# SimLeek/pySILEnT

Measured on AMD Instinct MI355X. Metric: Mpx/s full pyramid line-end pass @1080p, 1/2/4/8 GPU; % HBM roofline, higher is better.
Workload: dtype f32

## Files before the change

pysilent_amd/csrc/silent_common.h:

```cpp
#pragma once

#include <hip/hip_runtime.h>
#include <stdint.h>

#include <type_traits>

#include "../../include/silent_hip.h"

namespace silent {

constexpr int kMaxLevels = SILENT_MAX_LEVELS;
constexpr int kWave = 64;

struct LevelTab {
    int n_levels;
    int tiles_per_frame;
    long long frame_px;
    int h[kMaxLevels];
    int w[kMaxLevels];
    int tiles_x[kMaxLevels];
    int tile_start[kMaxLevels + 1];
    long long px_off[kMaxLevels];
};

constexpr int kChunk = 1024;

struct TileCoord {
    int frame, level, ty, tx;
};

__device__ __forceinline__ unsigned xcd_swizzle(unsigned bid, unsigned n) {
    constexpr unsigned kXcd = 8;
    const unsigned per = n / kXcd, rem = n % kXcd;
    const unsigned x = bid % kXcd, k = bid / kXcd;
    return x * per + (x < rem ? x : rem) + k;
}

__device__ __forceinline__ TileCoord locate_tile(const LevelTab& tab, unsigned bid) {
    TileCoord t;
    t.frame = (int)(bid / (unsigned)tab.tiles_per_frame);
    int rem = (int)(bid - (unsigned)t.frame * (unsigned)tab.tiles_per_frame);
    int l = 0;
#pragma unroll
    for (int i = 1; i < kMaxLevels; ++i)
        if (i < tab.n_levels && rem >= tab.tile_start[i]) l = i;
    t.level = l;
    rem -= tab.tile_start[l];
    t.ty = rem / tab.tiles_x[l];
    t.tx = rem - t.ty * tab.tiles_x[l];
    return t;
}

__device__ __forceinline__ float from_lane_below(float v) {
    return __int_as_float(__builtin_amdgcn_update_dpp(0, __float_as_int(v), 0x138 , 0xf, 0xf, true));
}
__device__ __forceinline__ float from_lane_above(float v) {
    return __int_as_float(__builtin_amdgcn_update_dpp(0, __float_as_int(v), 0x130 , 0xf, 0xf, true));
}

template <bool F64>
using acc_t = typename std::conditional<F64, double, float>::type;
__device__ __forceinline__ double bpermute_f64(int addr, double v) {
    return __hiloint2double(__builtin_amdgcn_ds_bpermute(addr, __double2hiint(v)), __builtin_amdgcn_ds_bpermute(addr, __double2loint(v)));
}

constexpr int kMirrorNearMin = 5;
__device__ __forceinline__ int mirror_near(int i, int n) {
    i = i < 0 ? -i : i;
    i = i >= n ? 2 * (n - 1) - i : i;
    return min(max(i, 0), n - 1);
}

template <bool EDGE = true>
__device__ __forceinline__ float unit_taps6(float c0, float edge, const float (&w)[6]) {
    const float l1 = from_lane_below(c0), l2 = from_lane_below(l1);
    float r1;
    if constexpr (EDGE)
        r1 = __int_as_float(__builtin_amdgcn_update_dpp(__float_as_int(edge), __float_as_int(c0), 0x130 , 0xf, 0xf, false));
    else
        r1 = from_lane_above(c0);
    const float r2 = from_lane_above(r1), r3 = from_lane_above(r2);
    float h = w[0] * l2;
    h = __builtin_fmaf(w[1], l1, h);
    h = __builtin_fmaf(w[2], c0, h);
    h = __builtin_fmaf(w[3], r1, h);
    h = __builtin_fmaf(w[4], r2, h);
    return __builtin_fmaf(w[5], r3, h);
}
template <bool EDGE = true>
__device__ __forceinline__ double unit_taps6(float c0, float edge, const double (&w)[6]) {
// ... 139 lines not shown
```

pysilent_amd/csrc/silent_gray.h:

```cpp
#pragma once

#include "silent_common.h"

namespace silent {

struct GrayW {
    float cs[9];
    float end[9 * 8];
};

constexpr int kGrayCols = 60;
constexpr int kGrayTW = 4 * kGrayCols;
constexpr int kGrayTH = 16;

template <bool NT = false>
__device__ __forceinline__ void store_row_k8(float* __restrict__ row_base ,
                                             const float (&acc)[8], float* s_slab ,
                                             int lane, int first, int count) {
    typedef float nf4 __attribute__((ext_vector_type(4)));
    nf4* slab4 = reinterpret_cast<nf4*>(s_slab);
    slab4[lane * 2 + 0] = nf4{acc[0], acc[1], acc[2], acc[3]};
    slab4[lane * 2 + 1] = nf4{acc[4], acc[5], acc[6], acc[7]};
    __builtin_amdgcn_wave_barrier();
    const nf4 a = slab4[lane], b = slab4[64 + lane];
// ... 42 lines not shown
#define SILENT_F16_CS_PAIRED 1
#endif
template <bool NT>
__device__ __forceinline__ void store_cs_row(gray_half* __restrict__ row0, float v, int lane, int first, int count) {
    const gray_half h = (gray_half)v;
    const unsigned mine = (unsigned)__builtin_bit_cast(unsigned short, h);
    const bool own = lane >= first && lane < first + count;
#if SILENT_F16_CS_PAIRED
    const unsigned up = (unsigned)__builtin_amdgcn_update_dpp(0, (int)mine, 0x130 , 0xf, 0xf, true);
    const int odd0 = (int)((reinterpret_cast<unsigned long long>(row0) >> 1) & 1ull);
    const bool lead = ((lane + odd0) & 1) == 0;
    const bool pair = own && lead && lane + 1 < first + count;
    const bool single = own && (lead ? lane + 1 >= first + count : lane == first);
    if (pair) {
        unsigned* p = reinterpret_cast<unsigned*>(row0 + lane);
        if constexpr (NT) __builtin_nontemporal_store(mine | (up << 16), p);
        else *p = mine | (up << 16);
    }
    if (single) {
        unsigned short* p = reinterpret_cast<unsigned short*>(row0 + lane);
        if constexpr (NT) __builtin_nontemporal_store((unsigned short)mine, p);
        else *p = (unsigned short)mine;
    }
#else
    if (own) {
        unsigned short* p = reinterpret_cast<unsigned short*>(row0 + lane);
        if constexpr (NT) __builtin_nontemporal_store((unsigned short)mine, p);
        else *p = (unsigned short)mine;
    }
#endif
}
template <typename ST>
constexpr bool kStoreHalf = std::is_same<ST, gray_half>::value;

struct GrayKp {
    unsigned* mm;
    float* sum;
    int* nan_flags;
    float* value_out;
    long long sum_frame;
    long long sum_off[kMaxLevels];
    int n_levels, pad, gpt;
    int level[kMaxLevels];
};

struct GrayKpAcc {
    float mx = kPoolLowest, nmn = kPoolLowest, grp = kPoolLowest;
    bool nan = false;
};

template <int K>
__device__ __forceinline__ void gray_kp_pixel(const GrayKp& kp, const float (&acc)[K], int y, int x, int H, int W, bool valid,
                                              float* __restrict__ value_px, GrayKpAcc& a) {
    const float m = (y >= kp.pad && y < H - kp.pad && x >= kp.pad && x < W - kp.pad) ? 1.0f : 0.0f;
    float s = __fmul_rn(m, acc[0]);
#pragma unroll
    for (int k = 1; k < K; ++k) s = __fadd_rn(s, __fmul_rn(m, acc[k]));
    const float v = __fmul_rn(s, 1.0f / (float)K);
    if (valid) {
        a.mx = pool_max(a.mx, v);
        a.nmn = pool_max(a.nmn, -v);
        a.grp = pool_max(a.grp, v);
        a.nan = a.nan || v != v;
        if (kp.value_out) *value_px = v;
    }
}
// ... 446 lines not shown
    if constexpr (F64) return stream_col64(st, g, wx_tile, lane);
    else return stream_col(st, g, wx_tile, lane);
}
template <int L, int G, int GR, int PR>
__device__ __forceinline__ void stream_level_f64(int g, const int (&cur)[PR], float c0, double (&vacc)[kStreamSlots],
                                                 const StreamCol64 (&col)[GR > 0 ? GR : 1], const StreamTab& st, int wx_tile, int lane,
                                                 float* __restrict__ pyr, long long frame_px0, int C, int ch) {
    const int meta = cur[g];
#pragma unroll
    for (int k = 0; k < stream_slots(L, g); ++k) {
        const int e = stream_w_off(L, G, g, true) + 2 * k;
        const double w = __hiloint2double(cur[e + 1], cur[e]);
        const double prev = (meta >> k) & 1 ? 0.0 : vacc[k];
        vacc[k] = __builtin_fma(w, (double)c0, prev);
    }
    const int done = (meta >> stream_done_shift(L)) & 7;
    if (done != 7) {
        const int oy = meta >> stream_row_shift(L);
        double v = vacc[0];
#pragma unroll
        for (int k = 1; k < stream_slots(L, g); ++k) v = done == k ? vacc[k] : v;
        const StreamCol64 cr = g < GR ? col[g < GR ? g : 0] : stream_col64(st, g, wx_tile, lane);
        double acc = cr.w[0] * bpermute_f64(cr.lane4, v);
#pragma unroll
        for (int t = 1; t < 6; ++t) acc = __builtin_fma(cr.w[t], bpermute_f64(cr.lane4 + 4 * t, v), acc);
        if (lane < cr.n) pyr[(frame_px0 + st.px_off[g] + (long long)oy * st.out_w[g] + cr.x0 + lane) * C + ch] = (float)acc;
    }
}
#ifndef SILENT_STREAM_REG_LEVELS
#define SILENT_STREAM_REG_LEVELS 3
#endif
constexpr int kStreamRegLevels = SILENT_STREAM_REG_LEVELS;

template <int K, int G, int L = 0, bool KP = false, bool F64 = false, typename ST = float, typename FT = float>
__global__ __launch_bounds__(64 * kFusedWaves) void gray_stream_kernel(frame_param<FT> frames, float* __restrict__ pyr,
                                                          ST* __restrict__ cs_out, ST* __restrict__ end_out,
                                                          const FusedTabT<F64> tab, const StreamTab st, const GrayW wts,
                                                          float clip_hi, unsigned opts, const GrayKp kp = GrayKp{}) {
    constexpr int R = kFusedTH, NR = kStreamRows;
    static_assert(!kStoreHalf<ST> || (!KP && !F64), "float16 storage: no keypoint epilogue, no float64 accumulation");
    static_assert(kFrameType<FT> && (!kFrameNarrow<FT> || !F64), "uint8 / uint16 frames: float32 accumulation only");
    __shared__ __attribute__((aligned(16))) float s_slab[K == 8 && !kStoreHalf<ST> ? kFusedWaves * 512 : 4];
    __shared__ __attribute__((aligned(16))) float s_rows[kFusedWaves][NR][64];
    const unsigned bid = (opts & 1u) ? xcd_swizzle(blockIdx.x, gridDim.x) : blockIdx.x;
    const int frame = (int)(bid / (unsigned)tab.tiles_per_frame);
    const int rem = (int)(bid - (unsigned)frame * (unsigned)tab.tiles_per_frame);
    const FusedLevel& lv = tab.lv[0];
    const int ty = rem / lv.tiles_x, tx = rem - ty * lv.tiles_x;

    const int lane = threadIdx.x & 63;
    const int wave = __builtin_amdgcn_readfirstlane(threadIdx.x >> 6);
    const int xw0 = tx * kFusedTW + wave * kFusedCols;
    const bool live = xw0 < lv.out_w;
    const int wx_tile = tx * kFusedWaves + wave;
    const int y0 = ty * R;
    const int ox = xw0 + lane - 4;
    const int W = tab.W;
    frame_src<FT> src;
    if constexpr (kFrameStrided<FT>) src = frame_of(frames, frame);
    else src = frames + (long long)frame * tab.H * W;
    const long long frame_px0 = (long long)frame * tab.frame_px;
    const long long base_px = frame_px0 + lv.px_off;

    const long long sx = mirror_near(ox, lv.src_w) + lv.src_x0;
    float in[R + 8];
    float in_last = 0.0f, xcol = 0.0f;
    constexpr int GR = G < kStreamRegLevels ? G : kStreamRegLevels;
    StreamColT<F64> col[GR > 0 ? GR : 1];
#pragma unroll
    for (int i = 0; i < R + 8; ++i) in[i] = 0.0f;
#pragma unroll
    for (int g = 0; g < GR; ++g) {
        col[g].x0 = col[g].n = col[g].lane4 = 0;
#pragma unroll
        for (int j = 0; j < 6; ++j) col[g].w[j] = 0.0f;
    }
    if (live) {
#pragma unroll
        for (int i = 0; i < R + 8; ++i)
        {
            if constexpr (kFrameStrided<FT>) in[i] = src.at(mirror_near(y0 - 4 + i, lv.src_h) + lv.src_y0, sx);
            else in[i] = (float)src[(long long)(mirror_near(y0 - 4 + i, lv.src_h) + lv.src_y0) * W + sx];
        }
        if constexpr (kFrameStrided<FT>) in_last = src.at(mirror_near(y0 + R + 4, lv.src_h) + lv.src_y0, sx);
        else in_last = (float)src[(long long)(mirror_near(y0 + R + 4, lv.src_h) + lv.src_y0) * W + sx];
        xcol = unit_edge_column(src, W, xw0 + 60, lv.src_w, lv.src_x0, y0 - 4, R + 9, lv.src_h, lv.src_y0, lane);
#pragma unroll
        for (int g = 0; g < GR; ++g) col[g] = stream_col_t<F64>(st, g, wx_tile, lane);
    }
    if (!live) return;
#pragma unroll
    for (int i = 0; i < R + 8; ++i) asm volatile("" ::"v"(in[i]));
    asm volatile("" : "+v"(in_last), "+v"(xcol));
#pragma unroll
    for (int g = 0; g < GR; ++g) {
        asm volatile("" ::"v"(col[g].lane4));
#pragma unroll
        for (int j = 0; j < 6; ++j) asm volatile("" ::"v"(col[g].w[j]));
    }
#pragma unroll
    for (int i = 0; i < R + 8; ++i) s_rows[wave][i][lane] = in[i];

    acc_t<F64> vacc[G][kStreamSlots];
#pragma unroll
    for (int g = 0; g < G; ++g)
#pragma unroll
        for (int k = 0; k < kStreamSlots; ++k) vacc[g][k] = 0.0f;
    static_assert(G == stream_pad_levels(G), "row programs are padded to 4 or 7 levels");
    constexpr int PR = kStreamProgRow(L, G, F64);
    typedef const __attribute__((address_space(4))) int* const_int_ptr;
    const_int_ptr prog = (const_int_ptr)(st.row_prog + (long long)ty * (NR * PR));
    int cur[PR], nxt[PR];
#pragma unroll
    for (int e = 0; e < PR; ++e) cur[e] = prog[e];
    float c0 = s_rows[wave][0][lane];
    const int nr_run = NR;
#pragma unroll 1
    for (int i = 0; i < nr_run; ++i) {
        const int in = min(i + 1, NR - 1);
#pragma unroll
        for (int e = 0; e < PR; ++e) nxt[e] = prog[in * PR + e];
        const float c_next = s_rows[wave][in][lane];
#pragma unroll
        for (int g = 0; g < G; ++g) {
            const int meta = cur[g];
            if (!(meta & 128)) continue;
            if constexpr (F64) {
                stream_level_f64<L, G, GR>(g, cur, c0, vacc[g], col, st, wx_tile, lane, pyr, frame_px0, 1, 0);
            } else {
#pragma unroll
                for (int k = 0; k < stream_slots(L, g); ++k) {
                    const float w = __int_as_float(cur[stream_w_off(L, G, g) + k]);
                    const float prev = (meta >> k) & 1 ? 0.0f : vacc[g][k];
                    vacc[g][k] = __builtin_fmaf(w, c0, prev);
                }
                const int done = (meta >> stream_done_shift(L)) & 7;
                if (done != 7) {
                    const int oy = meta >> stream_row_shift(L);
                    float v = vacc[g][0];
#pragma unroll
                    for (int k = 1; k < stream_slots(L, g); ++k) v = done == k ? vacc[g][k] : v;
                    const int vbits = __float_as_int(v);
                    const StreamCol cr = g < GR ? col[g < GR ? g : 0] : stream_col(st, g, wx_tile, lane);
                    float acc = cr.w[0] * __int_as_float(__builtin_amdgcn_ds_bpermute(cr.lane4, vbits));
#pragma unroll
                    for (int t = 1; t < 6; ++t)
                        acc = __builtin_fmaf(cr.w[t], __int_as_float(__builtin_amdgcn_ds_bpermute(cr.lane4 + 4 * t, vbits)), acc);
                    if (lane < cr.n) pyr[frame_px0 + st.px_off[g] + (long long)oy * st.out_w[g] + cr.x0 + lane] = acc;
                }
            }
        }
#pragma unroll
        for (int e = 0; e < PR; ++e) cur[e] = nxt[e];
        c0 = c_next;
    }

    constexpr bool VW = K <= 4;
    acc_t<F64> wv[6];
    float csw[9], endw[VW ? 9 * K : 1];
#pragma unroll
    for (int j = 0; j < 6; ++j) {
        if constexpr (F64) wv[j] = tab.w64[j];
        else wv[j] = tab.wx[j];
        if constexpr (VW) asm volatile("" : "+v"(wv[j]));
    }
#pragma unroll
    for (int j = 0; j < 9; ++j) {
        csw[j] = wts.cs[j];
        if constexpr (VW) asm volatile("" : "+v"(csw[j]));
    }
    if constexpr (VW) {
#pragma unroll
        for (int j = 0; j < 9 * K; ++j) {
            endw[j] = wts.end[j];
            asm volatile("" : "+v"(endw[j]));
        }
    }
    const int eff_h = min(lv.zoom_h, lv.out_h), eff_w = min(lv.zoom_w, lv.out_w);
    const bool col_eff = ox >= 0 && ox < eff_w;
    const bool col_in = ox >= 0 && ox < lv.out_w;
    const bool out_lane = lane >= 4 && lane < 4 + kFusedCols && ox < lv.out_w;
    const long long wave_px = base_px + (xw0 - 4);
    {
        GrayKpAcc ka;
        acc_t<F64> hw[6] = {0, 0, 0, 0, 0, 0};
        float iw[3][3], cw[3][3];
#pragma unroll
        for (int a = 0; a < 3; ++a)
#pragma unroll
            for (int b = 0; b < 3; ++b) iw[a][b] = cw[a][b] = 0.0f;
#pragma unroll
        for (int i = 0; i < R + 9; ++i) {
            {
                const float c0 = i < R + 8 ? s_rows[wave][i < R + 8 ? i : 0][lane] : in_last;
                const acc_t<F64> h = unit_taps6(c0, unit_edge(xcol, i), wv);
#pragma unroll
                for (int j = 0; j < 5; ++j) hw[j] = hw[j + 1];
                hw[5] = h;
            }
            if (i >= 5) {
                const int p = y0 + i - 7;
                float v;
                if constexpr (F64) {
                    v = unit_vsum_f64(wv, hw);
                } else {
                    v = wv[0] * hw[0];
#pragma unroll
                    for (int j = 1; j < 6; ++j) v = __builtin_fmaf(wv[j], hw[j], v);
                }
                v = (p >= 0 && p < eff_h && col_eff) ? v : 0.0f;
                if (p >= y0 && p < y0 + R && p < lv.out_h) {
                    float* __restrict__ prow = pyr + (wave_px + (long long)p * lv.out_w);
                    if (out_lane) __builtin_nontemporal_store(v, prow + lane);
                }
#pragma unroll
                for (int b = 0; b < 3; ++b) {
                    iw[0][b] = iw[1][b];
                    iw[1][b] = iw[2][b];
                }
                iw[2][1] = v;
                iw[2][0] = from_lane_below(v);
                iw[2][2] = from_lane_above(v);
            }
            if (i >= 7) {
                const int c = y0 + i - 8;
                float acc = 0.0f;
                if constexpr (F64) {
                    acc = gray_cs_f64(iw, csw);
                } else {
#pragma unroll
                    for (int dy = 0; dy < 3; ++dy)
#pragma unroll
                        for (int dx = 0; dx < 3; ++dx) acc = __builtin_fmaf(iw[dy][dx], csw[dy * 3 + dx], acc);
                }
                const float cs = (c >= 0 && c < lv.out_h && col_in && !(acc < 0.0f)) ? acc : 0.0f;
#pragma unroll
                for (int b = 0; b < 3; ++b) {
                    cw[0][b] = cw[1][b];
                    cw[1][b] = cw[2][b];
                }
                cw[2][1] = cs;
                cw[2][0] = from_lane_below(cs);
                cw[2][2] = from_lane_above(cs);
            }
            if (i >= 9) {
                const int y = y0 + i - 9;
                if (y < lv.out_h) {
                    const long long row_px = wave_px + (long long)y * lv.out_w;
                    if constexpr (kStoreHalf<ST>) {
                        if (cs_out) store_cs_row<true>(cs_out + row_px, cw[1][1], lane, 4, min(kFusedCols, lv.out_w - xw0));
                    } else if (cs_out) {
                        float* __restrict__ crow = cs_out + row_px;
                        if (out_lane) __builtin_nontemporal_store(cw[1][1], crow + lane);
                    }
                    if (end_out) {
                        float acc[K];
                        if constexpr (F64) {
                            gray_end_f64<K>(cw, VW ? endw : wts.end, clip_hi, acc);
                        } else {
#pragma unroll
                            for (int k = 0; k < K; ++k) acc[k] = 0.0f;
#pragma unroll
                            for (int dy = 0; dy < 3; ++dy)
#pragma unroll
                                for (int dx = 0; dx < 3; ++dx)
#pragma unroll
                                    for (int k = 0; k < K; ++k) {
                                        const int wi = (dy * 3 + dx) * K + k;
                                        if constexpr (VW) acc[k] = __builtin_fmaf(cw[dy][dx], endw[wi], acc[k]);
                                        else acc[k] = __builtin_fmaf(cw[dy][dx], wts.end[wi], acc[k]);
                                    }
                            relu_clip_tf(acc, clip_hi);
                        }
                        if constexpr (KP) gray_kp_pixel<K>(kp, acc, y, ox, lv.out_h, lv.out_w, out_lane, kp.value_out + row_px + lane, ka);
                        if constexpr (K == 8) {
                            const int ncols = min(kFusedCols, lv.out_w - xw0);
                            store_row_k8<true>(end_out + row_px * 8, acc, s_slab + wave * 512, lane, 4, ncols);
                        } else if constexpr (kStoreHalf<ST>) {
                            if (out_lane) store_end_px<K, K == 4>(end_out + (row_px + lane) * K, acc);
                        } else if constexpr (K == 4) {
                            typedef float nf4 __attribute__((ext_vector_type(4)));
                            nf4* __restrict__ erow = reinterpret_cast<nf4*>(end_out + row_px * 4);
                            if (out_lane) __builtin_nontemporal_store(nf4{acc[0], acc[1], acc[2], acc[3]}, erow + lane);
                        } else {
                            float* __restrict__ po = end_out + row_px * K;
                            if (out_lane) {
#pragma unroll
                                for (int k = 0; k < K; ++k) po[lane * K + k] = acc[k];
                            }
                        }
                    }
                }
                if constexpr (KP) {
                    if (kp_group_ends(i - 9, R)) gray_kp_group_end(kp, ka, frame, kp.level[0], ty, (i - 9) / kSumRows, ox, lv.out_w, out_lane);
                }
            }
        }
        if constexpr (KP) gray_kp_tile_end(kp, ka, frame, kp.level[0], lane);
    }
}

template <int C, int G, int L = 0, bool F64 = false, typename FT = float>
__global__ __launch_bounds__(64 * kFusedWaves) void pyramid_stream_kernel(frame_param<FT> frames, float* __restrict__ pyr,
                                                             const FusedTabT<F64> tab, const StreamTab st) {
    static_assert(kFrameType<FT> && (!kFrameNarrow<FT> || (!F64 && C == 1)), "uint8 / uint16 frames: one channel, float32 accumulation");
    constexpr int R = kFusedTH, NR = kStreamRows;
    __shared__ float s_rows[kFusedWaves][NR][64];
    const unsigned bid = blockIdx.x;
    const int frame = (int)(bid / (unsigned)tab.tiles_per_frame);
    const int rem = (int)(bid - (unsigned)frame * (unsigned)tab.tiles_per_frame);
    const FusedLevel& lv = tab.lv[0];
    const int ty = rem / lv.tiles_x, tx = rem - ty * lv.tiles_x;
    const int lane = threadIdx.x & 63;
    const int wave = __builtin_amdgcn_readfirstlane(threadIdx.x >> 6);
    const int xw0 = tx * kFusedTW + wave * kFusedCols;
    if (xw0 >= lv.out_w) return;
    const int wx_tile = tx * kFusedWaves + wave;
    const int y0 = ty * R;
    const int ox = xw0 + lane - 4;
    const long long WC = (long long)tab.W * C;
    frame_src<FT> src;
    if constexpr (kFrameStrided<FT>) src = frame_of(frames, frame);
    else src = frames + (long long)frame * tab.H * WC;
    const long long frame_px0 = (long long)frame * tab.frame_px;
    const long long base_px = frame_px0 + lv.px_off;
    const long long sx = (long long)(mirror_near(ox, lv.src_w) + lv.src_x0) * C;

    constexpr int GR = G < kStreamRegLevels ? G : kStreamRegLevels;
    StreamColT<F64> col[GR > 0 ? GR : 1];
#pragma unroll
    for (int g = 0; g < GR; ++g) col[g] = stream_col_t<F64>(st, g, wx_tile, lane);
// ... 100 lines not shown
```

Measured before the change: 135,800.

## Split gray stream kernel into interior and border tile bodies

```diff
diff --git a/pysilent_amd/csrc/silent_common.h b/pysilent_amd/csrc/silent_common.h
--- a/pysilent_amd/csrc/silent_common.h
+++ b/pysilent_amd/csrc/silent_common.h
@@ -56,6 +56,14 @@
 }
 __device__ __forceinline__ float from_lane_above(float v) {
     return __int_as_float(__builtin_amdgcn_update_dpp(0, __float_as_int(v), 0x130 , 0xf, 0xf, true));
+}
+
+template <typename T>
+using global_ptr = __attribute__((address_space(1))) T*;
+template <typename T>
+__device__ __forceinline__ void advance_rows(global_ptr<T>& p, long long elements) {
+    p += elements;
+    asm("" : "+s"(p));
 }
 
 template <bool F64>
diff --git a/pysilent_amd/csrc/silent_gray.h b/pysilent_amd/csrc/silent_gray.h
--- a/pysilent_amd/csrc/silent_gray.h
+++ b/pysilent_amd/csrc/silent_gray.h
@@ -98,6 +98,18 @@
 }
 template <typename ST>
 constexpr bool kStoreHalf = std::is_same<ST, gray_half>::value;
+template <int K, typename ST>
+__device__ __forceinline__ void store_end_lane(ST* __restrict__ row0, int lane, const float (&acc)[K]) {
+    if constexpr (kStoreHalf<ST>) {
+        store_end_px<K, K == 4>(row0 + lane * K, acc);
+    } else if constexpr (K == 4) {
+        typedef float nf4 __attribute__((ext_vector_type(4)));
+        __builtin_nontemporal_store(nf4{acc[0], acc[1], acc[2], acc[3]}, reinterpret_cast<nf4*>(row0) + lane);
+    } else {
+#pragma unroll
+        for (int k = 0; k < K; ++k) row0[lane * K + k] = acc[k];
+    }
+}
 
 struct GrayKp {
     unsigned* mm;
@@ -610,271 +622,42 @@
 #endif
 constexpr int kStreamRegLevels = SILENT_STREAM_REG_LEVELS;
 
+template <int K, int G>
+constexpr bool kStreamTwoBodies = K == 4 && G <= 4;
+
+template <bool INTERIOR, int K, int G, int L, bool KP, bool F64, typename ST, typename FT>
+__device__ __forceinline__ void gray_stream_tile(frame_param<FT> frames, float* __restrict__ pyr, ST* __restrict__ cs_out,
+                                                 ST* __restrict__ end_out, const FusedTabT<F64> tab, const StreamTab st, const GrayW wts,
+                                                 float clip_hi, const GrayKp kp, float* s_slab, float (*s_rows)[kStreamRows][64],
+                                                 int frame, int ty, int tx, int wave, int lane) {
+#include "silent_gray_stream_tile.h"
+}
+
 template <int K, int G, int L = 0, bool KP = false, bool F64 = false, typename ST = float, typename FT = float>
 __global__ __launch_bounds__(64 * kFusedWaves) void gray_stream_kernel(frame_param<FT> frames, float* __restrict__ pyr,
                                                           ST* __restrict__ cs_out, ST* __restrict__ end_out,
                                                           const FusedTabT<F64> tab, const StreamTab st, const GrayW wts,
                                                           float clip_hi, unsigned opts, const GrayKp kp = GrayKp{}) {
-    constexpr int R = kFusedTH, NR = kStreamRows;
     static_assert(!kStoreHalf<ST> || (!KP && !F64), "float16 storage: no keypoint epilogue, no float64 accumulation");
     static_assert(kFrameType<FT> && (!kFrameNarrow<FT> || !F64), "uint8 / uint16 frames: float32 accumulation only");
     __shared__ __attribute__((aligned(16))) float s_slab[K == 8 && !kStoreHalf<ST> ? kFusedWaves * 512 : 4];
-    __shared__ __attribute__((aligned(16))) float s_rows[kFusedWaves][NR][64];
+    __shared__ __attribute__((aligned(16))) float s_rows[kFusedWaves][kStreamRows][64];
     const unsigned bid = (opts & 1u) ? xcd_swizzle(blockIdx.x, gridDim.x) : blockIdx.x;
     const int frame = (int)(bid / (unsigned)tab.tiles_per_frame);
     const int rem = (int)(bid - (unsigned)frame * (unsigned)tab.tiles_per_frame);
-    const FusedLevel& lv = tab.lv[0];
-    const int ty = rem / lv.tiles_x, tx = rem - ty * lv.tiles_x;
-
+    const int ty = rem / tab.lv[0].tiles_x, tx = rem - ty * tab.lv[0].tiles_x;
     const int lane = threadIdx.x & 63;
     const int wave = __builtin_amdgcn_readfirstlane(threadIdx.x >> 6);
-    const int xw0 = tx * kFusedTW + wave * kFusedCols;
-    const bool live = xw0 < lv.out_w;
-    const int wx_tile = tx * kFusedWaves + wave;
-    const int y0 = ty * R;
-    const int ox = xw0 + lane - 4;
-    const int W = tab.W;
-    frame_src<FT> src;
-    if constexpr (kFrameStrided<FT>) src = frame_of(frames, frame);
-    else src = frames + (long long)frame * tab.H * W;
-    const long long frame_px0 = (long long)frame * tab.frame_px;
-    const long long base_px = frame_px0 + lv.px_off;
-
-    const long long sx = mirror_near(ox, lv.src_w) + lv.src_x0;
-    float in[R + 8];
-    float in_last = 0.0f, xcol = 0.0f;
-    constexpr int GR = G < kStreamRegLevels ? G : kStreamRegLevels;
-    StreamColT<F64> col[GR > 0 ? GR : 1];
-#pragma unroll
-    for (int i = 0; i < R + 8; ++i) in[i] = 0.0f;
-#pragma unroll
-    for (int g = 0; g < GR; ++g) {
-        col[g].x0 = col[g].n = col[g].lane4 = 0;
-#pragma unroll
-        for (int j = 0; j < 6; ++j) col[g].w[j] = 0.0f;
-    }
-    if (live) {
-#pragma unroll
-        for (int i = 0; i < R + 8; ++i)
-        {
-            if constexpr (kFrameStrided<FT>) in[i] = src.at(mirror_near(y0 - 4 + i, lv.src_h) + lv.src_y0, sx);
-            else in[i] = (float)src[(long long)(mirror_near(y0 - 4 + i, lv.src_h) + lv.src_y0) * W + sx];
-        }
-        if constexpr (kFrameStrided<FT>) in_last = src.at(mirror_near(y0 + R + 4, lv.src_h) + lv.src_y0, sx);
-        else in_last = (float)src[(long long)(mirror_near(y0 + R + 4, lv.src_h) + lv.src_y0) * W + sx];
-        xcol = unit_edge_column(src, W, xw0 + 60, lv.src_w, lv.src_x0, y0 - 4, R + 9, lv.src_h, lv.src_y0, lane);
-#pragma unroll
-        for (int g = 0; g < GR; ++g) col[g] = stream_col_t<F64>(st, g, wx_tile, lane);
-    }
-    if (!live) return;
-#pragma unroll
-    for (int i = 0; i < R + 8; ++i) asm volatile("" ::"v"(in[i]));
-    asm volatile("" : "+v"(in_last), "+v"(xcol));
-#pragma unroll
-    for (int g = 0; g < GR; ++g) {
-        asm volatile("" ::"v"(col[g].lane4));
-#pragma unroll
-        for (int j = 0; j < 6; ++j) asm volatile("" ::"v"(col[g].w[j]));
-    }
-#pragma unroll
-    for (int i = 0; i < R + 8; ++i) s_rows[wave][i][lane] = in[i];
-
-    acc_t<F64> vacc[G][kStreamSlots];
-#pragma unroll
-    for (int g = 0; g < G; ++g)
-#pragma unroll
-        for (int k = 0; k < kStreamSlots; ++k) vacc[g][k] = 0.0f;
-    static_assert(G == stream_pad_levels(G), "row programs are padded to 4 or 7 levels");
-    constexpr int PR = kStreamProgRow(L, G, F64);
-    typedef const __attribute__((address_space(4))) int* const_int_ptr;
-    const_int_ptr prog = (const_int_ptr)(st.row_prog + (long long)ty * (NR * PR));
-    int cur[PR], nxt[PR];
-#pragma unroll
-    for (int e = 0; e < PR; ++e) cur[e] = prog[e];
-    float c0 = s_rows[wave][0][lane];
-    const int nr_run = NR;
-#pragma unroll 1
-    for (int i = 0; i < nr_run; ++i) {
-        const int in = min(i + 1, NR - 1);
-#pragma unroll
-        for (int e = 0; e < PR; ++e) nxt[e] = prog[in * PR + e];
-        const float c_next = s_rows[wave][in][lane];
-#pragma unroll
-        for (int g = 0; g < G; ++g) {
-            const int meta = cur[g];
-            if (!(meta & 128)) continue;
-            if constexpr (F64) {
-                stream_level_f64<L, G, GR>(g, cur, c0, vacc[g], col, st, wx_tile, lane, pyr, frame_px0, 1, 0);
-            } else {
-#pragma unroll
-                for (int k = 0; k < stream_slots(L, g); ++k) {
-                    const float w = __int_as_float(cur[stream_w_off(L, G, g) + k]);
-                    const float prev = (meta >> k) & 1 ? 0.0f : vacc[g][k];
-                    vacc[g][k] = __builtin_fmaf(w, c0, prev);
-                }
-                const int done = (meta >> stream_done_shift(L)) & 7;
-                if (done != 7) {
-                    const int oy = meta >> stream_row_shift(L);
-                    float v = vacc[g][0];
-#pragma unroll
-                    for (int k = 1; k < stream_slots(L, g); ++k) v = done == k ? vacc[g][k] : v;
-                    const int vbits = __float_as_int(v);
-                    const StreamCol cr = g < GR ? col[g < GR ? g : 0] : stream_col(st, g, wx_tile, lane);
-                    float acc = cr.w[0] * __int_as_float(__builtin_amdgcn_ds_bpermute(cr.lane4, vbits));
-#pragma unroll
-                    for (int t = 1; t < 6; ++t)
-                        acc = __builtin_fmaf(cr.w[t], __int_as_float(__builtin_amdgcn_ds_bpermute(cr.lane4 + 4 * t, vbits)), acc);
-                    if (lane < cr.n) pyr[frame_px0 + st.px_off[g] + (long long)oy * st.out_w[g] + cr.x0 + lane] = acc;
-                }
-            }
-        }
-#pragma unroll
-        for (int e = 0; e < PR; ++e) cur[e] = nxt[e];
-        c0 = c_next;
-    }
-
-    constexpr bool VW = K <= 4;
-    acc_t<F64> wv[6];
-    float csw[9], endw[VW ? 9 * K : 1];
-#pragma unroll
-    for (int j = 0; j < 6; ++j) {
-        if constexpr (F64) wv[j] = tab.w64[j];
-        else wv[j] = tab.wx[j];
-        if constexpr (VW) asm volatile("" : "+v"(wv[j]));
-    }
-#pragma unroll
-    for (int j = 0; j < 9; ++j) {
-        csw[j] = wts.cs[j];
-        if constexpr (VW) asm volatile("" : "+v"(csw[j]));
-    }
-    if constexpr (VW) {
-#pragma unroll
-        for (int j = 0; j < 9 * K; ++j) {
-            endw[j] = wts.end[j];
-            asm volatile("" : "+v"(endw[j]));
-        }
-    }
-    const int eff_h = min(lv.zoom_h, lv.out_h), eff_w = min(lv.zoom_w, lv.out_w);
-    const bool col_eff = ox >= 0 && ox < eff_w;
-    const bool col_in = ox >= 0 && ox < lv.out_w;
-    const bool out_lane = lane >= 4 && lane < 4 + kFusedCols && ox < lv.out_w;
-    const long long wave_px = base_px + (xw0 - 4);
-    {
-        GrayKpAcc ka;
-        acc_t<F64> hw[6] = {0, 0, 0, 0, 0, 0};
-        float iw[3][3], cw[3][3];
-#pragma unroll
-        for (int a = 0; a < 3; ++a)
-#pragma unroll
-            for (int b = 0; b < 3; ++b) iw[a][b] = cw[a][b] = 0.0f;
-#pragma unroll
-        for (int i = 0; i < R + 9; ++i) {
-            {
-                const float c0 = i < R + 8 ? s_rows[wave][i < R + 8 ? i : 0][lane] : in_last;
-                const acc_t<F64> h = unit_taps6(c0, unit_edge(xcol, i), wv);
-#pragma unroll
-                for (int j = 0; j < 5; ++j) hw[j] = hw[j + 1];
-                hw[5] = h;
-            }
-            if (i >= 5) {
-                const int p = y0 + i - 7;
-                float v;
-                if constexpr (F64) {
-                    v = unit_vsum_f64(wv, hw);
-                } else {
-                    v = wv[0] * hw[0];
-#pragma unroll
-                    for (int j = 1; j < 6; ++j) v = __builtin_fmaf(wv[j], hw[j], v);
-                }
-                v = (p >= 0 && p < eff_h && col_eff) ? v : 0.0f;
-                if (p >= y0 && p < y0 + R && p < lv.out_h) {
-                    float* __restrict__ prow = pyr + (wave_px + (long long)p * lv.out_w);
-                    if (out_lane) __builtin_nontemporal_store(v, prow + lane);
-                }
-#pragma unroll
-                for (int b = 0; b < 3; ++b) {
-                    iw[0][b] = iw[1][b];
-                    iw[1][b] = iw[2][b];
-                }
-                iw[2][1] = v;
-                iw[2][0] = from_lane_below(v);
-                iw[2][2] = from_lane_above(v);
-            }
-            if (i >= 7) {
-                const int c = y0 + i - 8;
-                float acc = 0.0f;
-                if constexpr (F64) {
-                    acc = gray_cs_f64(iw, csw);
-                } else {
-#pragma unroll
-                    for (int dy = 0; dy < 3; ++dy)
-#pragma unroll
-                        for (int dx = 0; dx < 3; ++dx) acc = __builtin_fmaf(iw[dy][dx], csw[dy * 3 + dx], acc);
-                }
-                const float cs = (c >= 0 && c < lv.out_h && col_in && !(acc < 0.0f)) ? acc : 0.0f;
-#pragma unroll
-                for (int b = 0; b < 3; ++b) {
-                    cw[0][b] = cw[1][b];
-                    cw[1][b] = cw[2][b];
-                }
-                cw[2][1] = cs;
-                cw[2][0] = from_lane_below(cs);
-                cw[2][2] = from_lane_above(cs);
-            }
-            if (i >= 9) {
-                const int y = y0 + i - 9;
-                if (y < lv.out_h) {
-                    const long long row_px = wave_px + (long long)y * lv.out_w;
-                    if constexpr (kStoreHalf<ST>) {
-                        if (cs_out) store_cs_row<true>(cs_out + row_px, cw[1][1], lane, 4, min(kFusedCols, lv.out_w - xw0));
-                    } else if (cs_out) {
-                        float* __restrict__ crow = cs_out + row_px;
-                        if (out_lane) __builtin_nontemporal_store(cw[1][1], crow + lane);
-                    }
-                    if (end_out) {
-                        float acc[K];
-                        if constexpr (F64) {
-                            gray_end_f64<K>(cw, VW ? endw : wts.end, clip_hi, acc);
-                        } else {
-#pragma unroll
-                            for (int k = 0; k < K; ++k) acc[k] = 0.0f;
-#pragma unroll
-                            for (int dy = 0; dy < 3; ++dy)
-#pragma unroll
-                                for (int dx = 0; dx < 3; ++dx)
-#pragma unroll
-                                    for (int k = 0; k < K; ++k) {
-                                        const int wi = (dy * 3 + dx) * K + k;
-                                        if constexpr (VW) acc[k] = __builtin_fmaf(cw[dy][dx], endw[wi], acc[k]);
-                                        else acc[k] = __builtin_fmaf(cw[dy][dx], wts.end[wi], acc[k]);
-                                    }
-                            relu_clip_tf(acc, clip_hi);
-                        }
-                        if constexpr (KP) gray_kp_pixel<K>(kp, acc, y, ox, lv.out_h, lv.out_w, out_lane, kp.value_out + row_px + lane, ka);
-                        if constexpr (K == 8) {
-                            const int ncols = min(kFusedCols, lv.out_w - xw0);
-                            store_row_k8<true>(end_out + row_px * 8, acc, s_slab + wave * 512, lane, 4, ncols);
-                        } else if constexpr (kStoreHalf<ST>) {
-                            if (out_lane) store_end_px<K, K == 4>(end_out + (row_px + lane) * K, acc);
-                        } else if constexpr (K == 4) {
-                            typedef float nf4 __attribute__((ext_vector_type(4)));
-                            nf4* __restrict__ erow = reinterpret_cast<nf4*>(end_out + row_px * 4);
-                            if (out_lane) __builtin_nontemporal_store(nf4{acc[0], acc[1], acc[2], acc[3]}, erow + lane);
-                        } else {
-                            float* __restrict__ po = end_out + row_px * K;
-                            if (out_lane) {
-#pragma unroll
-                                for (int k = 0; k < K; ++k) po[lane * K + k] = acc[k];
-                            }
-                        }
-                    }
-                }
-                if constexpr (KP) {
-                    if (kp_group_ends(i - 9, R)) gray_kp_group_end(kp, ka, frame, kp.level[0], ty, (i - 9) / kSumRows, ox, lv.out_w, out_lane);
-                }
-            }
-        }
-        if constexpr (KP) gray_kp_tile_end(kp, ka, frame, kp.level[0], lane);
+    if constexpr (kStreamTwoBodies<K, G>) {
+        const FusedLevel& u = tab.lv[0];
+        const int wy0 = ty * kFusedTH, wx0 = tx * kFusedTW + wave * kFusedCols;
+        const int lim_h = min(u.src_h, min(u.zoom_h, u.out_h)), lim_w = min(u.src_w, min(u.zoom_w, u.out_w));
+        if (wy0 >= 4 && wy0 + kFusedTH + 4 < lim_h && wx0 >= 4 && wx0 + 60 < lim_w)
+            gray_stream_tile<true, K, G, L, KP, F64, ST, FT>(frames, pyr, cs_out, end_out, tab, st, wts, clip_hi, kp, s_slab, s_rows, frame, ty, tx, wave, lane);
+        else
+            gray_stream_tile<false, K, G, L, KP, F64, ST, FT>(frames, pyr, cs_out, end_out, tab, st, wts, clip_hi, kp, s_slab, s_rows, frame, ty, tx, wave, lane);
+    } else {
+#include "silent_gray_stream_tile_general.h"
     }
 }
 
diff --git a/pysilent_amd/csrc/silent_gray_stream_tile.h b/pysilent_amd/csrc/silent_gray_stream_tile.h
--- /dev/null
+++ b/pysilent_amd/csrc/silent_gray_stream_tile.h
@@ -0,0 +1,278 @@
+    constexpr int R = kFusedTH, NR = kStreamRows;
+    const FusedLevel& lv = tab.lv[0];
+    const int xw0 = tx * kFusedTW + wave * kFusedCols;
+    const bool live = xw0 < lv.out_w;
+    const int wx_tile = tx * kFusedWaves + wave;
+    const int y0 = ty * R;
+    const int ox = xw0 + lane - 4;
+    const int W = tab.W;
+    frame_src<FT> src;
+    if constexpr (kFrameStrided<FT>) src = frame_of(frames, frame);
+    else src = frames + (long long)frame * tab.H * W;
+    const long long frame_px0 = (long long)frame * tab.frame_px;
+    const long long base_px = frame_px0 + lv.px_off;
+
+    float in[R + 8];
+    float in_last = 0.0f, xcol = 0.0f;
+    constexpr int GR = G < kStreamRegLevels ? G : kStreamRegLevels;
+    StreamColT<F64> col[GR > 0 ? GR : 1];
+    if constexpr (INTERIOR) {
+        const int sy0 = y0 - 4 + lv.src_y0, sx0 = xw0 - 4 + lv.src_x0;
+        if constexpr (kFrameStrided<FT>) {
+            auto row = src;
+            global_ptr<const unsigned char> rp = (global_ptr<const unsigned char>)(src.p + (sy0 * src.row_stride + sx0 * src.pixel_stride));
+#pragma unroll
+            for (int i = 0; i < R + 9; ++i) {
+                row.p = (const unsigned char*)rp;
+                const float f = row.at(0, lane);
+                if (i < R + 8) in[i < R + 8 ? i : 0] = f;
+                else in_last = f;
+                advance_rows(rp, src.row_stride);
+            }
+            xcol = src.at(sy0 + min(lane, R + 8), sx0 + 64);
+        } else {
+            global_ptr<const FT> rp = (global_ptr<const FT>)(src + ((long long)sy0 * W + sx0));
+#pragma unroll
+            for (int i = 0; i < R + 9; ++i) {
+                const float f = (float)((const FT*)rp)[lane];
+                if (i < R + 8) in[i < R + 8 ? i : 0] = f;
+                else in_last = f;
+                advance_rows(rp, W);
+            }
+            xcol = (float)src[(long long)(sy0 + min(lane, R + 8)) * W + (sx0 + 64)];
+        }
+#pragma unroll
+        for (int g = 0; g < GR; ++g) col[g] = stream_col_t<F64>(st, g, wx_tile, lane);
+    } else {
+        const long long sx = mirror_near(ox, lv.src_w) + lv.src_x0;
+#pragma unroll
+        for (int i = 0; i < R + 8; ++i) in[i] = 0.0f;
+#pragma unroll
+        for (int g = 0; g < GR; ++g) {
+            col[g].x0 = col[g].n = col[g].lane4 = 0;
+#pragma unroll
+            for (int j = 0; j < 6; ++j) col[g].w[j] = 0.0f;
+        }
+        if (live) {
+#pragma unroll
+            for (int i = 0; i < R + 8; ++i)
+            {
+                if constexpr (kFrameStrided<FT>) in[i] = src.at(mirror_near(y0 - 4 + i, lv.src_h) + lv.src_y0, sx);
+                else in[i] = (float)src[(long long)(mirror_near(y0 - 4 + i, lv.src_h) + lv.src_y0) * W + sx];
+            }
+            if constexpr (kFrameStrided<FT>) in_last = src.at(mirror_near(y0 + R + 4, lv.src_h) + lv.src_y0, sx);
+            else in_last = (float)src[(long long)(mirror_near(y0 + R + 4, lv.src_h) + lv.src_y0) * W + sx];
+            xcol = unit_edge_column(src, W, xw0 + 60, lv.src_w, lv.src_x0, y0 - 4, R + 9, lv.src_h, lv.src_y0, lane);
+#pragma unroll
+            for (int g = 0; g < GR; ++g) col[g] = stream_col_t<F64>(st, g, wx_tile, lane);
+        }
+        if (!live) return;
+    }
+#pragma unroll
+    for (int i = 0; i < R + 8; ++i) asm volatile("" ::"v"(in[i]));
+    asm volatile("" : "+v"(in_last), "+v"(xcol));
+#pragma unroll
+    for (int g = 0; g < GR; ++g) {
+        asm volatile("" ::"v"(col[g].lane4));
+#pragma unroll
+        for (int j = 0; j < 6; ++j) asm volatile("" ::"v"(col[g].w[j]));
+    }
+#pragma unroll
+    for (int i = 0; i < R + 8; ++i) s_rows[wave][i][lane] = in[i];
+
+    acc_t<F64> vacc[G][kStreamSlots];
+#pragma unroll
+    for (int g = 0; g < G; ++g)
+#pragma unroll
+        for (int k = 0; k < kStreamSlots; ++k) vacc[g][k] = 0.0f;
+    static_assert(G == stream_pad_levels(G), "row programs are padded to 4 or 7 levels");
+    constexpr int PR = kStreamProgRow(L, G, F64);
+    typedef const __attribute__((address_space(4))) int* const_int_ptr;
+    const_int_ptr prog = (const_int_ptr)(st.row_prog + (long long)ty * (NR * PR));
+    static_assert(NR % 2 == 0, "pass 2 runs two stream rows per iteration");
+    constexpr int HS = 2;
+    int rec[2][PR];
+    float cv[2];
+#pragma unroll
+    for (int e = 0; e < PR; ++e) rec[0][e] = prog[e];
+    cv[0] = s_rows[wave][0][lane];
+#pragma unroll 1
+    for (int i = 0; i < NR; i += HS) {
+#pragma unroll
+        for (int h = 0; h < HS; ++h) {
+            const int (&cur)[PR] = rec[h];
+            const float c0 = cv[h];
+            const int in = min(i + h + 1, NR - 1);
+#pragma unroll
+            for (int e = 0; e < PR; ++e) rec[h ^ 1][e] = prog[in * PR + e];
+            cv[h ^ 1] = s_rows[wave][in][lane];
+#pragma unroll
+            for (int g = 0; g < G; ++g) {
+                const int meta = cur[g];
+                if (!(meta & 128)) continue;
+                if constexpr (F64) {
+                    stream_level_f64<L, G, GR>(g, cur, c0, vacc[g], col, st, wx_tile, lane, pyr, frame_px0, 1, 0);
+                } else {
+#pragma unroll
+                    for (int k = 0; k < stream_slots(L, g); ++k) {
+                        const float w = __int_as_float(cur[stream_w_off(L, G, g) + k]);
+                        const float prev = (meta >> k) & 1 ? 0.0f : vacc[g][k];
+                        vacc[g][k] = __builtin_fmaf(w, c0, prev);
+                    }
+                    const int done = (meta >> stream_done_shift(L)) & 7;
+                    if (done != 7) {
+                        const int oy = meta >> stream_row_shift(L);
+                        float v = vacc[g][0];
+#pragma unroll
+                        for (int k = 1; k < stream_slots(L, g); ++k) v = done == k ? vacc[g][k] : v;
+                        const int vbits = __float_as_int(v);
+                        const StreamCol cr = g < GR ? col[g < GR ? g : 0] : stream_col(st, g, wx_tile, lane);
+                        float acc = cr.w[0] * __int_as_float(__builtin_amdgcn_ds_bpermute(cr.lane4, vbits));
+#pragma unroll
+                        for (int t = 1; t < 6; ++t)
+                            acc = __builtin_fmaf(cr.w[t], __int_as_float(__builtin_amdgcn_ds_bpermute(cr.lane4 + 4 * t, vbits)), acc);
+                        if (lane < cr.n) pyr[frame_px0 + st.px_off[g] + (long long)oy * st.out_w[g] + cr.x0 + lane] = acc;
+                    }
+                }
+            }
+        }
+    }
+
+    constexpr bool VW = K <= 4;
+    acc_t<F64> wv[6];
+    float csw[9], endw[VW ? 9 * K : 1];
+#pragma unroll
+    for (int j = 0; j < 6; ++j) {
+        if constexpr (F64) wv[j] = tab.w64[j];
+        else wv[j] = tab.wx[j];
+        if constexpr (VW) asm volatile("" : "+v"(wv[j]));
+    }
+#pragma unroll
+    for (int j = 0; j < 9; ++j) {
+        csw[j] = wts.cs[j];
+        if constexpr (VW) asm volatile("" : "+v"(csw[j]));
+    }
+    if constexpr (VW) {
+#pragma unroll
+        for (int j = 0; j < 9 * K; ++j) {
+            endw[j] = wts.end[j];
+            asm volatile("" : "+v"(endw[j]));
+        }
+    }
+    const int eff_h = min(lv.zoom_h, lv.out_h), eff_w = min(lv.zoom_w, lv.out_w);
+    const bool col_eff = INTERIOR || (ox >= 0 && ox < eff_w);
+    const bool col_in = INTERIOR || (ox >= 0 && ox < lv.out_w);
+    const bool out_lane = lane >= 4 && lane < 4 + kFusedCols && (INTERIOR || ox < lv.out_w);
+    const long long wave_px = base_px + (xw0 - 4);
+    global_ptr<float> prow = (global_ptr<float>)(pyr + (wave_px + (long long)y0 * lv.out_w));
+    global_ptr<ST> crow = (global_ptr<ST>)(cs_out + (wave_px + (long long)y0 * lv.out_w));
+    global_ptr<ST> erow = (global_ptr<ST>)(end_out + (wave_px + (long long)y0 * lv.out_w) * K);
+    {
+        GrayKpAcc ka;
+        acc_t<F64> hw[6] = {0, 0, 0, 0, 0, 0};
+        float iw[3][3], cw[3][3];
+#pragma unroll
+        for (int a = 0; a < 3; ++a)
+#pragma unroll
+            for (int b = 0; b < 3; ++b) iw[a][b] = cw[a][b] = 0.0f;
+#pragma unroll
+        for (int i = 0; i < R + 9; ++i) {
+            {
+                const float c0 = i < R + 8 ? s_rows[wave][i < R + 8 ? i : 0][lane] : in_last;
+                const acc_t<F64> h = unit_taps6(c0, unit_edge(xcol, i), wv);
+#pragma unroll
+                for (int j = 0; j < 5; ++j) hw[j] = hw[j + 1];
+                hw[5] = h;
+            }
+            if (i >= 5) {
+                const int p = y0 + i - 7;
+                float v;
+                if constexpr (F64) {
+                    v = unit_vsum_f64(wv, hw);
+                } else {
+                    v = wv[0] * hw[0];
+#pragma unroll
+                    for (int j = 1; j < 6; ++j) v = __builtin_fmaf(wv[j], hw[j], v);
+                }
+                if constexpr (!INTERIOR) v = (p >= 0 && p < eff_h && col_eff) ? v : 0.0f;
+                if (p >= y0 && p < y0 + R && (INTERIOR || p < lv.out_h)) {
+                    if (out_lane) __builtin_nontemporal_store(v, (float*)prow + lane);
+                    advance_rows(prow, lv.out_w);
+                }
+#pragma unroll
+                for (int b = 0; b < 3; ++b) {
+                    iw[0][b] = iw[1][b];
+                    iw[1][b] = iw[2][b];
+                }
+                iw[2][1] = v;
+                iw[2][0] = from_lane_below(v);
+                iw[2][2] = from_lane_above(v);
+            }
+            if (i >= 7) {
+                const int c = y0 + i - 8;
+                float acc = 0.0f;
+                if constexpr (F64) {
+                    acc = gray_cs_f64(iw, csw);
+                } else {
+#pragma unroll
+                    for (int dy = 0; dy < 3; ++dy)
+#pragma unroll
+                        for (int dx = 0; dx < 3; ++dx) acc = __builtin_fmaf(iw[dy][dx], csw[dy * 3 + dx], acc);
+                }
+                const float cs = (INTERIOR || (c >= 0 && c < lv.out_h && col_in)) && !(acc < 0.0f) ? acc : 0.0f;
+#pragma unroll
+                for (int b = 0; b < 3; ++b) {
+                    cw[0][b] = cw[1][b];
+                    cw[1][b] = cw[2][b];
+                }
+                cw[2][1] = cs;
+                cw[2][0] = from_lane_below(cs);
+                cw[2][2] = from_lane_above(cs);
+            }
+            if (i >= 9) {
+                const int y = y0 + i - 9;
+                if (INTERIOR || y < lv.out_h) {
+                    ST* __restrict__ crow_y = (ST*)crow;
+                    ST* __restrict__ erow_y = (ST*)erow;
+                    if constexpr (kStoreHalf<ST>) {
+                        if (cs_out) store_cs_row<true>(crow_y, cw[1][1], lane, 4, INTERIOR ? kFusedCols : min(kFusedCols, lv.out_w - xw0));
+                    } else if (cs_out) {
+                        if (out_lane) __builtin_nontemporal_store(cw[1][1], crow_y + lane);
+                    }
+                    if (end_out) {
+                        float acc[K];
+                        if constexpr (F64) {
+                            gray_end_f64<K>(cw, VW ? endw : wts.end, clip_hi, acc);
+                        } else {
+#pragma unroll
+                            for (int k = 0; k < K; ++k) acc[k] = 0.0f;
+#pragma unroll
+                            for (int dy = 0; dy < 3; ++dy)
+#pragma unroll
+                                for (int dx = 0; dx < 3; ++dx)
+#pragma unroll
+                                    for (int k = 0; k < K; ++k) {
+                                        const int wi = (dy * 3 + dx) * K + k;
+                                        if constexpr (VW) acc[k] = __builtin_fmaf(cw[dy][dx], endw[wi], acc[k]);
+                                        else acc[k] = __builtin_fmaf(cw[dy][dx], wts.end[wi], acc[k]);
+                                    }
+                            relu_clip_tf(acc, clip_hi);
+                        }
+                        if constexpr (KP) gray_kp_pixel<K>(kp, acc, y, ox, lv.out_h, lv.out_w, out_lane, kp.value_out + (wave_px + (long long)y * lv.out_w) + lane, ka);
+                        if constexpr (K == 8) {
+                            const int ncols = INTERIOR ? kFusedCols : min(kFusedCols, lv.out_w - xw0);
+                            store_row_k8<true>(erow_y, acc, s_slab + wave * 512, lane, 4, ncols);
+                        } else {
+                            if (out_lane) store_end_lane<K>(erow_y, lane, acc);
+                        }
+                    }
+                    advance_rows(crow, lv.out_w);
+                    advance_rows(erow, (long long)lv.out_w * K);
+                }
+                if constexpr (KP) {
+                    if (kp_group_ends(i - 9, R)) gray_kp_group_end(kp, ka, frame, kp.level[0], ty, (i - 9) / kSumRows, ox, lv.out_w, out_lane);
+                }
+            }
+        }
+        if constexpr (KP) gray_kp_tile_end(kp, ka, frame, kp.level[0], lane);
+    }
diff --git a/pysilent_amd/csrc/silent_gray_stream_tile_general.h b/pysilent_amd/csrc/silent_gray_stream_tile_general.h
--- /dev/null
+++ b/pysilent_amd/csrc/silent_gray_stream_tile_general.h
@@ -0,0 +1,250 @@
+    constexpr int R = kFusedTH, NR = kStreamRows;
+    const FusedLevel& lv = tab.lv[0];
+    const int xw0 = tx * kFusedTW + wave * kFusedCols;
+    const bool live = xw0 < lv.out_w;
+    const int wx_tile = tx * kFusedWaves + wave;
+    const int y0 = ty * R;
+    const int ox = xw0 + lane - 4;
+    const int W = tab.W;
+    frame_src<FT> src;
+    if constexpr (kFrameStrided<FT>) src = frame_of(frames, frame);
+    else src = frames + (long long)frame * tab.H * W;
+    const long long frame_px0 = (long long)frame * tab.frame_px;
+    const long long base_px = frame_px0 + lv.px_off;
+
+    const long long sx = mirror_near(ox, lv.src_w) + lv.src_x0;
+    float in[R + 8];
+    float in_last = 0.0f, xcol = 0.0f;
+    constexpr int GR = G < kStreamRegLevels ? G : kStreamRegLevels;
+    StreamColT<F64> col[GR > 0 ? GR : 1];
+#pragma unroll
+    for (int i = 0; i < R + 8; ++i) in[i] = 0.0f;
+#pragma unroll
+    for (int g = 0; g < GR; ++g) {
+        col[g].x0 = col[g].n = col[g].lane4 = 0;
+#pragma unroll
+        for (int j = 0; j < 6; ++j) col[g].w[j] = 0.0f;
+    }
+    if (live) {
+#pragma unroll
+        for (int i = 0; i < R + 8; ++i)
+        {
+            if constexpr (kFrameStrided<FT>) in[i] = src.at(mirror_near(y0 - 4 + i, lv.src_h) + lv.src_y0, sx);
+            else in[i] = (float)src[(long long)(mirror_near(y0 - 4 + i, lv.src_h) + lv.src_y0) * W + sx];
+        }
+        if constexpr (kFrameStrided<FT>) in_last = src.at(mirror_near(y0 + R + 4, lv.src_h) + lv.src_y0, sx);
+        else in_last = (float)src[(long long)(mirror_near(y0 + R + 4, lv.src_h) + lv.src_y0) * W + sx];
+        xcol = unit_edge_column(src, W, xw0 + 60, lv.src_w, lv.src_x0, y0 - 4, R + 9, lv.src_h, lv.src_y0, lane);
+#pragma unroll
+        for (int g = 0; g < GR; ++g) col[g] = stream_col_t<F64>(st, g, wx_tile, lane);
+    }
+    if (!live) return;
+#pragma unroll
+    for (int i = 0; i < R + 8; ++i) asm volatile("" ::"v"(in[i]));
+    asm volatile("" : "+v"(in_last), "+v"(xcol));
+#pragma unroll
+    for (int g = 0; g < GR; ++g) {
+        asm volatile("" ::"v"(col[g].lane4));
+#pragma unroll
+        for (int j = 0; j < 6; ++j) asm volatile("" ::"v"(col[g].w[j]));
+    }
+#pragma unroll
+    for (int i = 0; i < R + 8; ++i) s_rows[wave][i][lane] = in[i];
+
+    acc_t<F64> vacc[G][kStreamSlots];
+#pragma unroll
+    for (int g = 0; g < G; ++g)
+#pragma unroll
+        for (int k = 0; k < kStreamSlots; ++k) vacc[g][k] = 0.0f;
+    static_assert(G == stream_pad_levels(G), "row programs are padded to 4 or 7 levels");
+    constexpr int PR = kStreamProgRow(L, G, F64);
+    typedef const __attribute__((address_space(4))) int* const_int_ptr;
+    const_int_ptr prog = (const_int_ptr)(st.row_prog + (long long)ty * (NR * PR));
+    int cur[PR], nxt[PR];
+#pragma unroll
+    for (int e = 0; e < PR; ++e) cur[e] = prog[e];
+    float c0 = s_rows[wave][0][lane];
+    const int nr_run = NR;
+#pragma unroll 1
+    for (int i = 0; i < nr_run; ++i) {
+        const int in = min(i + 1, NR - 1);
+#pragma unroll
+        for (int e = 0; e < PR; ++e) nxt[e] = prog[in * PR + e];
+        const float c_next = s_rows[wave][in][lane];
+#pragma unroll
+        for (int g = 0; g < G; ++g) {
+            const int meta = cur[g];
+            if (!(meta & 128)) continue;
+            if constexpr (F64) {
+                stream_level_f64<L, G, GR>(g, cur, c0, vacc[g], col, st, wx_tile, lane, pyr, frame_px0, 1, 0);
+            } else {
+#pragma unroll
+                for (int k = 0; k < stream_slots(L, g); ++k) {
+                    const float w = __int_as_float(cur[stream_w_off(L, G, g) + k]);
+                    const float prev = (meta >> k) & 1 ? 0.0f : vacc[g][k];
+                    vacc[g][k] = __builtin_fmaf(w, c0, prev);
+                }
+                const int done = (meta >> stream_done_shift(L)) & 7;
+                if (done != 7) {
+                    const int oy = meta >> stream_row_shift(L);
+                    float v = vacc[g][0];
+#pragma unroll
+                    for (int k = 1; k < stream_slots(L, g); ++k) v = done == k ? vacc[g][k] : v;
+                    const int vbits = __float_as_int(v);
+                    const StreamCol cr = g < GR ? col[g < GR ? g : 0] : stream_col(st, g, wx_tile, lane);
+                    float acc = cr.w[0] * __int_as_float(__builtin_amdgcn_ds_bpermute(cr.lane4, vbits));
+#pragma unroll
+                    for (int t = 1; t < 6; ++t)
+                        acc = __builtin_fmaf(cr.w[t], __int_as_float(__builtin_amdgcn_ds_bpermute(cr.lane4 + 4 * t, vbits)), acc);
+                    if (lane < cr.n) pyr[frame_px0 + st.px_off[g] + (long long)oy * st.out_w[g] + cr.x0 + lane] = acc;
+                }
+            }
+        }
+#pragma unroll
+        for (int e = 0; e < PR; ++e) cur[e] = nxt[e];
+        c0 = c_next;
+    }
+
+    constexpr bool VW = K <= 4;
+    acc_t<F64> wv[6];
+    float csw[9], endw[VW ? 9 * K : 1];
+#pragma unroll
+    for (int j = 0; j < 6; ++j) {
+        if constexpr (F64) wv[j] = tab.w64[j];
+        else wv[j] = tab.wx[j];
+        if constexpr (VW) asm volatile("" : "+v"(wv[j]));
+    }
+#pragma unroll
+    for (int j = 0; j < 9; ++j) {
+        csw[j] = wts.cs[j];
+        if constexpr (VW) asm volatile("" : "+v"(csw[j]));
+    }
+    if constexpr (VW) {
+#pragma unroll
+        for (int j = 0; j < 9 * K; ++j) {
+            endw[j] = wts.end[j];
+            asm volatile("" : "+v"(endw[j]));
+        }
+    }
+    const int eff_h = min(lv.zoom_h, lv.out_h), eff_w = min(lv.zoom_w, lv.out_w);
+    const bool col_eff = ox >= 0 && ox < eff_w;
+    const bool col_in = ox >= 0 && ox < lv.out_w;
+    const bool out_lane = lane >= 4 && lane < 4 + kFusedCols && ox < lv.out_w;
+    const long long wave_px = base_px + (xw0 - 4);
+    {
+        GrayKpAcc ka;
+        acc_t<F64> hw[6] = {0, 0, 0, 0, 0, 0};
+        float iw[3][3], cw[3][3];
+#pragma unroll
+        for (int a = 0; a < 3; ++a)
+#pragma unroll
+            for (int b = 0; b < 3; ++b) iw[a][b] = cw[a][b] = 0.0f;
+#pragma unroll
+        for (int i = 0; i < R + 9; ++i) {
+            {
+                const float c0 = i < R + 8 ? s_rows[wave][i < R + 8 ? i : 0][lane] : in_last;
+                const acc_t<F64> h = unit_taps6(c0, unit_edge(xcol, i), wv);
+#pragma unroll
+                for (int j = 0; j < 5; ++j) hw[j] = hw[j + 1];
+                hw[5] = h;
+            }
+            if (i >= 5) {
+                const int p = y0 + i - 7;
+                float v;
+                if constexpr (F64) {
+                    v = unit_vsum_f64(wv, hw);
+                } else {
+                    v = wv[0] * hw[0];
+#pragma unroll
+                    for (int j = 1; j < 6; ++j) v = __builtin_fmaf(wv[j], hw[j], v);
+                }
+                v = (p >= 0 && p < eff_h && col_eff) ? v : 0.0f;
+                if (p >= y0 && p < y0 + R && p < lv.out_h) {
+                    float* __restrict__ prow = pyr + (wave_px + (long long)p * lv.out_w);
+                    if (out_lane) __builtin_nontemporal_store(v, prow + lane);
+                }
+#pragma unroll
+                for (int b = 0; b < 3; ++b) {
+                    iw[0][b] = iw[1][b];
+                    iw[1][b] = iw[2][b];
+                }
+                iw[2][1] = v;
+                iw[2][0] = from_lane_below(v);
+                iw[2][2] = from_lane_above(v);
+            }
+            if (i >= 7) {
+                const int c = y0 + i - 8;
+                float acc = 0.0f;
+                if constexpr (F64) {
+                    acc = gray_cs_f64(iw, csw);
+                } else {
+#pragma unroll
+                    for (int dy = 0; dy < 3; ++dy)
+#pragma unroll
+                        for (int dx = 0; dx < 3; ++dx) acc = __builtin_fmaf(iw[dy][dx], csw[dy * 3 + dx], acc);
+                }
+                const float cs = (c >= 0 && c < lv.out_h && col_in && !(acc < 0.0f)) ? acc : 0.0f;
+#pragma unroll
+                for (int b = 0; b < 3; ++b) {
+                    cw[0][b] = cw[1][b];
+                    cw[1][b] = cw[2][b];
+                }
+                cw[2][1] = cs;
+                cw[2][0] = from_lane_below(cs);
+                cw[2][2] = from_lane_above(cs);
+            }
+            if (i >= 9) {
+                const int y = y0 + i - 9;
+                if (y < lv.out_h) {
+                    const long long row_px = wave_px + (long long)y * lv.out_w;
+                    if constexpr (kStoreHalf<ST>) {
+                        if (cs_out) store_cs_row<true>(cs_out + row_px, cw[1][1], lane, 4, min(kFusedCols, lv.out_w - xw0));
+                    } else if (cs_out) {
+                        float* __restrict__ crow = cs_out + row_px;
+                        if (out_lane) __builtin_nontemporal_store(cw[1][1], crow + lane);
+                    }
+                    if (end_out) {
+                        float acc[K];
+                        if constexpr (F64) {
+                            gray_end_f64<K>(cw, VW ? endw : wts.end, clip_hi, acc);
+                        } else {
+#pragma unroll
+                            for (int k = 0; k < K; ++k) acc[k] = 0.0f;
+#pragma unroll
+                            for (int dy = 0; dy < 3; ++dy)
+#pragma unroll
+                                for (int dx = 0; dx < 3; ++dx)
+#pragma unroll
+                                    for (int k = 0; k < K; ++k) {
+                                        const int wi = (dy * 3 + dx) * K + k;
+                                        if constexpr (VW) acc[k] = __builtin_fmaf(cw[dy][dx], endw[wi], acc[k]);
+                                        else acc[k] = __builtin_fmaf(cw[dy][dx], wts.end[wi], acc[k]);
+                                    }
+                            relu_clip_tf(acc, clip_hi);
+                        }
+                        if constexpr (KP) gray_kp_pixel<K>(kp, acc, y, ox, lv.out_h, lv.out_w, out_lane, kp.value_out + row_px + lane, ka);
+                        if constexpr (K == 8) {
+                            const int ncols = min(kFusedCols, lv.out_w - xw0);
+                            store_row_k8<true>(end_out + row_px * 8, acc, s_slab + wave * 512, lane, 4, ncols);
+                        } else if constexpr (kStoreHalf<ST>) {
+                            if (out_lane) store_end_px<K, K == 4>(end_out + (row_px + lane) * K, acc);
+                        } else if constexpr (K == 4) {
+                            typedef float nf4 __attribute__((ext_vector_type(4)));
+                            nf4* __restrict__ erow = reinterpret_cast<nf4*>(end_out + row_px * 4);
+                            if (out_lane) __builtin_nontemporal_store(nf4{acc[0], acc[1], acc[2], acc[3]}, erow + lane);
+                        } else {
+                            float* __restrict__ po = end_out + row_px * K;
+                            if (out_lane) {
+#pragma unroll
+                                for (int k = 0; k < K; ++k) po[lane * K + k] = acc[k];
+                            }
+                        }
+                    }
+                }
+                if constexpr (KP) {
+                    if (kp_group_ends(i - 9, R)) gray_kp_group_end(kp, ka, frame, kp.level[0], ty, (i - 9) / kSumRows, ox, lv.out_w, out_lane);
+                }
+            }
+        }
+        if constexpr (KP) gray_kp_tile_end(kp, ka, frame, kp.level[0], lane);
+    }
```

Result: faster. 142,800 (median of 6 runs) (+5.2%).
